# yukara-ikemiya/friendly-stable-audio-tools

Measured on NVIDIA H100. Metric: denoise_steps_per_s, higher is better.
Workload: dtype fp16 operands, fp32 accumulate (the reference's autocast dtype)

## Files before the change

friendly-stable-audio-tools_b200/csrc/gemm.cuh:

```cuda
#pragma once
#include "common.cuh"
#include "ptx.cuh"

namespace satb {

__device__ __forceinline__ int split_part(int idx, int n_parts) { return n_parts == 3 ? (idx == 2 ? 0 : idx + 1) : idx; }

struct GemmShape {
  int L;
  int batches;
  int N;
  int K;
  int n_taps;
  int tap_base;
  int tap_step;
  int b_tap_rows;
  int stride;
  int b_static = 0;
  int n_parts = 1;
  int b_part_rows = 0;
};

constexpr int kBlockM = 128;
constexpr int kBlockK = 64;
constexpr int kWgmmaK = 16;
constexpr int kGemmThreads = 384;
constexpr int kSmemBudget = 227 * 1024;

constexpr int kEpiWarps = 8;
template <int BN, int kCols, int kEpiStage = 0>
struct GemmCfg {
  static constexpr int kStageA = kBlockM * kBlockK * 2;
  static constexpr int kStageB = BN * kBlockK * 2;
  static constexpr int kStage = kStageA + kStageB;
  static constexpr int kAccLd = kCols + 4;
  static constexpr int kAccStage = 2 * 64 * kAccLd * 4;
  static constexpr int kFixed = 1024  + 256  + 2 * kAccStage + kEpiWarps * kEpiStage;
  static constexpr int kStages = (kSmemBudget - kFixed) / kStage > 8 ? 8 : (kSmemBudget - kFixed) / kStage;
  static constexpr int kSmemBytes = kStages * kStage + kFixed;
  static_assert(BN == 64 || BN == 128 || BN == 256, "BN must be 64/128/256");
  static_assert(kStages >= 2, "shared memory too small for a two-stage ring");
};

struct EpiCtx {
  int row;
  int l;
  int batch;
  int col0;
  bool valid;
  int l0;
  int L;
  int lane;
  float* stage;
};

template <class Epi, int BN>
__device__ __forceinline__ void gemm_tile_epilogue(const float (&acc)[BN / 2], float* acc_st, float* epi_st,
                                                   const typename Epi::Params& ep, int L, int N, int m0, int n0, int batch,
                                                   int cw, int warp, int lane) {
  const int wq = warp & 3;
  const int half = wq >> 1;
  const int rsub = (wq & 1) * 32;
  const int fr = 16 * wq + (lane >> 2);
  const int fc = 2 * (lane & 3);
  constexpr int kChunks = BN / Epi::kCols;
  constexpr int kLd = Epi::kCols + 4;
  EpiCtx c;
  c.l0 = m0 + 64 * cw + rsub;
  c.l = c.l0 + lane;
  c.batch = batch;
  c.row = batch * L + c.l;
  c.valid = c.l < L;
  c.L = L;
  c.lane = lane;
  c.stage = epi_st;
  int n_valid = (N - n0 + Epi::kCols - 1) / Epi::kCols;
  if (n_valid > kChunks) n_valid = kChunks;
#pragma unroll
  for (int cp = 0; cp < (kChunks + 1) / 2; ++cp) {
    named_bar_sync(1 + cw, 128);
#pragma unroll
    for (int hh = 0; hh < 2; ++hh) {
      const int ch = 2 * cp + hh;
      if (ch < kChunks) {
        float* dst = acc_st + hh * 64 * kLd;
#pragma unroll
        for (int j = 0; j < Epi::kCols / 8; ++j) {
          const int ai = (ch * (Epi::kCols / 8) + j) * 4;
          *reinterpret_cast<float2*>(dst + fr * kLd + 8 * j + fc) = make_float2(acc[ai], acc[ai + 1]);
          *reinterpret_cast<float2*>(dst + (fr + 8) * kLd + 8 * j + fc) = make_float2(acc[ai + 2], acc[ai + 3]);
        }
      }
    }
    named_bar_sync(1 + cw, 128);
    const int ci = 2 * cp + half;
    if (ci < n_valid) {
      uint32_t r[Epi::kCols];
      const float4* src = reinterpret_cast<const float4*>(acc_st + half * 64 * kLd + (rsub + lane) * kLd);
#pragma unroll
      for (int j = 0; j < Epi::kCols / 4; ++j) {
        const float4 v = src[j];
        r[4 * j] = __float_as_uint(v.x);
        r[4 * j + 1] = __float_as_uint(v.y);
        r[4 * j + 2] = __float_as_uint(v.z);
        r[4 * j + 3] = __float_as_uint(v.w);
      }
      c.col0 = n0 + ci * Epi::kCols;
      Epi::apply(ep, c, r);
    }
  }
}
template <class Epi, int BN, bool BF16>
__global__ void __launch_bounds__(kGemmThreads, 1)
gemm_wgmma_kernel(const __grid_constant__ CUtensorMap tmA, const __grid_constant__ CUtensorMap tmB,
                  const __grid_constant__ CUtensorMap tmA2, const GemmShape s, const typename Epi::Params ep) {
  using Cfg = GemmCfg<BN, Epi::kCols, Epi::kStageBytes>;
  extern __shared__ uint8_t smem_raw[];
  uint8_t* smem = reinterpret_cast<uint8_t*>((reinterpret_cast<uintptr_t>(smem_raw) + 1023) & ~uintptr_t(1023));
  uint64_t* bars = reinterpret_cast<uint64_t*>(smem + Cfg::kStages * Cfg::kStage);
  uint64_t* full_bar = bars;
  uint64_t* empty_bar = bars + Cfg::kStages;
  uint8_t* epi_smem = smem + Cfg::kStages * Cfg::kStage + 256;

  const int warp = threadIdx.x >> 5;
  const int lane = threadIdx.x & 31;
  const int wg = threadIdx.x >> 7;

  const int m_tiles = (s.L + kBlockM - 1) / kBlockM;
  const int n_tiles = (s.N + BN - 1) / BN;
  const int tiles_per_n = m_tiles * s.batches;
  const int total_tiles = tiles_per_n * n_tiles;
  const int kb_per_tap = (s.K + kBlockK - 1) / kBlockK;
  const int kb_per_part = kb_per_tap * s.n_taps;
  const int num_kb = kb_per_part * s.n_parts;

  if (threadIdx.x == 0) {
    tma_prefetch_desc(&tmA);
    tma_prefetch_desc(&tmB);
    for (int i = 0; i < Cfg::kStages; ++i) {
      mbar_init(&full_bar[i], 1);
      mbar_init(&empty_bar[i], 2);
    }
    fence_mbar_init();
  }
  __syncthreads();
  pdl_launch_dependents();

  if (wg == 0) {
    setmaxnreg_dec<40>();
    if (warp == 0 && elect_one()) {
      int pre = 0;
      if (s.b_static && static_cast<int>(blockIdx.x) < total_tiles) {
        pre = num_kb < Cfg::kStages ? num_kb : Cfg::kStages;
        const int n0 = (static_cast<int>(blockIdx.x) / tiles_per_n) * BN;
        for (int kb = 0; kb < pre; ++kb) {
          const int pidx = kb / kb_per_part, kbp = kb - pidx * kb_per_part;
          const int part = split_part(pidx, s.n_parts);
          const int tap = kbp / kb_per_tap;
          const int k0 = (kbp - tap * kb_per_tap) * kBlockK;
          mbar_expect_tx(&full_bar[kb], Cfg::kStage);
          tma_load_2d(smem + kb * Cfg::kStage + Cfg::kStageA, &tmB, &full_bar[kb], k0,
                      tap * s.b_tap_rows + n0 + (part == 2 ? s.b_part_rows : 0));
        }
      }
      pdl_wait();
      int stage = 0;
      uint32_t phase = 0;
      for (int tile = blockIdx.x; tile < total_tiles; tile += gridDim.x) {
        const int nt = tile / tiles_per_n;
        const int rem = tile - nt * tiles_per_n;
        const int batch = rem / m_tiles;
        const int m0 = (rem - batch * m_tiles) * kBlockM;
        const int n0 = nt * BN;
        for (int kb = 0; kb < num_kb; ++kb) {
          const int pidx = kb / kb_per_part, kbp = kb - pidx * kb_per_part;
          const int part = split_part(pidx, s.n_parts);
          const int tap = kbp / kb_per_tap;
          const int k0 = (kbp - tap * kb_per_tap) * kBlockK;
          mbar_wait(&empty_bar[stage], phase ^ 1);
          uint8_t* sa = smem + stage * Cfg::kStage;
          uint8_t* sb = sa + Cfg::kStageA;
          const bool b_done = tile == static_cast<int>(blockIdx.x) && kb < pre;
          if (!b_done) mbar_expect_tx(&full_bar[stage], Cfg::kStage);
          const int u = s.tap_base + tap * s.tap_step;
          int ph = 0, ro = u;
          if (s.stride > 1) {
            ro = (u >= 0) ? u / s.stride : -((-u + s.stride - 1) / s.stride);
            ph = u - ro * s.stride;
          }
          tma_load_4d(sa, part == 1 ? &tmA2 : &tmA, &full_bar[stage], k0, ph, m0 + ro, batch);
          if (!b_done)
            tma_load_2d(sb, &tmB, &full_bar[stage], k0, tap * s.b_tap_rows + n0 + (part == 2 ? s.b_part_rows : 0));
          if (++stage == Cfg::kStages) {
            stage = 0;
            phase ^= 1;
          }
        }
      }
    }
  } else {
    setmaxnreg_inc<232>();
    pdl_wait();
    const int cw = wg - 1;
    float* acc_st = reinterpret_cast<float*>(epi_smem + cw * Cfg::kAccStage);
    float* epi_st = Epi::kStageBytes > 0
                        ? reinterpret_cast<float*>(epi_smem + 2 * Cfg::kAccStage + (warp - 4) * Epi::kStageBytes)
                        : nullptr;
    float acc[BN / 2];
    int stage = 0;
    uint32_t phase = 0;
    for (int tile = blockIdx.x; tile < total_tiles; tile += gridDim.x) {
      const int nt = tile / tiles_per_n;
      const int rem = tile - nt * tiles_per_n;
      const int batch = rem / m_tiles;
      const int m0 = (rem - batch * m_tiles) * kBlockM;
      const int n0 = nt * BN;
      int prev = -1;
      for (int kb = 0; kb < num_kb; ++kb) {
        mbar_wait(&full_bar[stage], phase);
        const uint32_t a_addr = smem_u32(smem + stage * Cfg::kStage) + cw * 64 * kBlockK * 2;
        const uint32_t b_addr = smem_u32(smem + stage * Cfg::kStage) + Cfg::kStageA;
        wgmma_fence();
#pragma unroll
        for (int k = 0; k < kBlockK / kWgmmaK; ++k)
          wgmma_ss<BN, BF16>(acc, make_desc_kmajor_sw128(a_addr + k * kWgmmaK * 2),
                             make_desc_kmajor_sw128(b_addr + k * kWgmmaK * 2), (kb | k) != 0 ? 1u : 0u);
        wgmma_commit();
        wgmma_wait<1>(acc);
        if (prev >= 0 && (threadIdx.x & 127) == 0) mbar_arrive(&empty_bar[prev]);
        prev = stage;
        if (++stage == Cfg::kStages) {
          stage = 0;
          phase ^= 1;
        }
      }
      wgmma_wait<0>(acc);
      if ((threadIdx.x & 127) == 0) mbar_arrive(&empty_bar[prev]);

      gemm_tile_epilogue<Epi, BN>(acc, acc_st, epi_st, ep, s.L, s.N, m0, n0, batch, cw, warp, lane);
    }
  }
}


__device__ __forceinline__ float silu_f(float x) { return x / (1.0f + __expf(-x)); }

template <bool BF16>
struct EpiStore16 {
  static constexpr int kCols = 32;
  static constexpr int kStageBytes = 0;
  struct Params {
    void* out;
    int ld;
    const float* bias;
    int act;
  };
  __device__ static __forceinline__ void apply(const Params& p, const EpiCtx& c, const uint32_t (&r)[32]) {
    if (!c.valid) return;
    float v[32];
#pragma unroll
    for (int j = 0; j < 32; ++j) v[j] = __uint_as_float(r[j]);
    if (p.bias) {
#pragma unroll
      for (int j = 0; j < 32; j += 4) {
        const float4 b = __ldg(reinterpret_cast<const float4*>(p.bias + c.col0 + j));
        v[j] += b.x; v[j + 1] += b.y; v[j + 2] += b.z; v[j + 3] += b.w;
      }
    }
    uint32_t o[16];
#pragma unroll
    for (int j = 0; j < 16; ++j) {
      float a = v[2 * j], b = v[2 * j + 1];
      if (p.act == 1) {
        a = silu_f(a);
        b = silu_f(b);
      }
      o[j] = Op16<BF16>::pack(a, b);
    }
    uint4* dst = reinterpret_cast<uint4*>(static_cast<uint16_t*>(p.out) + static_cast<size_t>(c.row) * p.ld + c.col0);
#pragma unroll
    for (int j = 0; j < 4; ++j) dst[j] = make_uint4(o[4 * j], o[4 * j + 1], o[4 * j + 2], o[4 * j + 3]);
  }
};

struct EpiStore32 {
  static constexpr int kCols = 32;
  static constexpr int kStageBytes = 0;
  struct Params {
    float* out;
    int ld;
    const float* bias;
  };
  __device__ static __forceinline__ void apply(const Params& p, const EpiCtx& c, const uint32_t (&r)[32]) {
    if (!c.valid) return;
    float4* dst = reinterpret_cast<float4*>(p.out + static_cast<size_t>(c.row) * p.ld + c.col0);
#pragma unroll
    for (int j = 0; j < 8; ++j) {
      float4 v = make_float4(__uint_as_float(r[4 * j]), __uint_as_float(r[4 * j + 1]), __uint_as_float(r[4 * j + 2]),
                             __uint_as_float(r[4 * j + 3]));
      if (p.bias) {
        const float4 b = __ldg(reinterpret_cast<const float4*>(p.bias + c.col0) + j);
        v.x += b.x; v.y += b.y; v.z += b.z; v.w += b.w;
      }
      dst[j] = v;
    }
  }
};

struct EpiResidual {
  static constexpr int kCols = 32;
  static constexpr int kStageBytes = 0;
  struct Params {
    float* h;
    int ld;
    const float* bias;
    const float* gate;
    int rows_per_item;
    int gate_ld;
    int n_items;
  };
  __device__ static __forceinline__ void apply(const Params& p, const EpiCtx& c, const uint32_t (&r)[32]) {
    if (!c.valid) return;
    float4* dst = reinterpret_cast<float4*>(p.h + static_cast<size_t>(c.row) * p.ld + c.col0);
    const float4* g = p.gate ? reinterpret_cast<const float4*>(
                                   p.gate + static_cast<size_t>((c.row / p.rows_per_item) % p.n_items) * p.gate_ld + c.col0)
                             : nullptr;
#pragma unroll
    for (int j = 0; j < 8; ++j) {
      float4 v = make_float4(__uint_as_float(r[4 * j]), __uint_as_float(r[4 * j + 1]), __uint_as_float(r[4 * j + 2]),
                             __uint_as_float(r[4 * j + 3]));
      if (p.bias) {
        const float4 b = __ldg(reinterpret_cast<const float4*>(p.bias + c.col0) + j);
        v.x += b.x; v.y += b.y; v.z += b.z; v.w += b.w;
      }
      if (g) {
        const float4 gg = __ldg(g + j);
        v.x *= gg.x; v.y *= gg.y; v.z *= gg.z; v.w *= gg.w;
      }
      asm volatile("red.global.add.v4.f32 [%0], {%1, %2, %3, %4};" ::"l"(dst + j), "f"(v.x), "f"(v.y), "f"(v.z), "f"(v.w)
                   : "memory");
    }
  }
};

template <bool BF16>
struct EpiQkvRope {
  static constexpr int kCols = 32;
  static constexpr int kStageBytes = 0;
  struct Params {
    void* out;
    int ld;
    int rope_cols;
    int seq_len;
    int head_dim;
    int nf;
    const float* cos_tab;
    const float* sin_tab;
  };
  __device__ static __forceinline__ void apply(const Params& p, const EpiCtx& c, const uint32_t (&r)[32]) {
    if (!c.valid) return;
    float v[32];
#pragma unroll
    for (int j = 0; j < 32; ++j) v[j] = __uint_as_float(r[j]);
    const int ci = (c.col0 % p.head_dim) >> 5;
    const int n_rot = min(max(p.nf - 16 * ci, 0), 16);
    if (c.col0 < p.rope_cols && n_rot > 0 && p.cos_tab) {
      const int pos = c.row % p.seq_len;
      const float4* ct = reinterpret_cast<const float4*>(p.cos_tab + pos * p.nf + 16 * ci);
      const float4* st = reinterpret_cast<const float4*>(p.sin_tab + pos * p.nf + 16 * ci);
#pragma unroll
      for (int j4 = 0; j4 < 4; ++j4) {
        if (4 * j4 >= n_rot) break;
        const float4 cs = __ldg(ct + j4), sn = __ldg(st + j4);
        const float cc[4] = {cs.x, cs.y, cs.z, cs.w}, ss[4] = {sn.x, sn.y, sn.z, sn.w};
#pragma unroll
        for (int u = 0; u < 4; ++u) {
          const int j = j4 * 4 + u;
          const float a = v[j], b = v[j + 16];
          v[j] = a * cc[u] - b * ss[u];
          v[j + 16] = b * cc[u] + a * ss[u];
        }
      }
    }
    uint4* dst = reinterpret_cast<uint4*>(static_cast<uint16_t*>(p.out) + static_cast<size_t>(c.row) * p.ld + c.col0);
#pragma unroll
    for (int j = 0; j < 4; ++j)
      dst[j] = make_uint4(Op16<BF16>::pack(v[8 * j], v[8 * j + 1]), Op16<BF16>::pack(v[8 * j + 2], v[8 * j + 3]),
                          Op16<BF16>::pack(v[8 * j + 4], v[8 * j + 5]), Op16<BF16>::pack(v[8 * j + 6], v[8 * j + 7]));
  }
};

template <bool BF16>
struct EpiHeadNorm16 {
  static constexpr int kCols = 64;
  static constexpr int kStageBytes = 0;
  struct Params {
    void* out;
    int ld;
    int norm_cols;
    int rope_cols;
    int seq_len;
    const float* cos_tab;
    const float* sin_tab;
  };
  __device__ static __forceinline__ void apply(const Params& p, const EpiCtx& c, const uint32_t (&r)[64]) {
    if (!c.valid) return;
    float inv = 1.f;
    if (c.col0 < p.norm_cols) {
      float ss = 0.f;
#pragma unroll
      for (int j = 0; j < 64; ++j) ss = fmaf(__uint_as_float(r[j]), __uint_as_float(r[j]), ss);
      inv = 1.f / fmaxf(sqrtf(ss), 1e-12f);
    }
    uint4* dst = reinterpret_cast<uint4*>(static_cast<uint16_t*>(p.out) + static_cast<size_t>(c.row) * p.ld + c.col0);
    float v[32];
#pragma unroll
    for (int j = 0; j < 32; ++j) v[j] = __uint_as_float(r[j]) * inv;
    if (c.col0 < p.rope_cols && p.cos_tab) {
      const int pos = c.row % p.seq_len;
      const float4* ct = reinterpret_cast<const float4*>(p.cos_tab + pos * 16);
      const float4* st = reinterpret_cast<const float4*>(p.sin_tab + pos * 16);
#pragma unroll
      for (int j4 = 0; j4 < 4; ++j4) {
        const float4 cs = __ldg(ct + j4), sn = __ldg(st + j4);
        const float cc[4] = {cs.x, cs.y, cs.z, cs.w}, ss4[4] = {sn.x, sn.y, sn.z, sn.w};
#pragma unroll
        for (int u = 0; u < 4; ++u) {
          const int j = j4 * 4 + u;
          const float a = v[j], b = v[j + 16];
          v[j] = a * cc[u] - b * ss4[u];
          v[j + 16] = b * cc[u] + a * ss4[u];
        }
      }
    }
#pragma unroll
    for (int j = 0; j < 4; ++j)
      dst[j] = make_uint4(Op16<BF16>::pack(v[8 * j], v[8 * j + 1]), Op16<BF16>::pack(v[8 * j + 2], v[8 * j + 3]),
                          Op16<BF16>::pack(v[8 * j + 4], v[8 * j + 5]), Op16<BF16>::pack(v[8 * j + 6], v[8 * j + 7]));
#pragma unroll
    for (int j = 0; j < 4; ++j) {
      const uint32_t* q = &r[32 + 8 * j];
      dst[4 + j] = make_uint4(Op16<BF16>::pack(__uint_as_float(q[0]) * inv, __uint_as_float(q[1]) * inv),
                              Op16<BF16>::pack(__uint_as_float(q[2]) * inv, __uint_as_float(q[3]) * inv),
                              Op16<BF16>::pack(__uint_as_float(q[4]) * inv, __uint_as_float(q[5]) * inv),
                              Op16<BF16>::pack(__uint_as_float(q[6]) * inv, __uint_as_float(q[7]) * inv));
    }
  }
};

template <bool BF16>
struct EpiSwiglu {
  static constexpr int kCols = 64;
  static constexpr int kStageBytes = 0;
  struct Params {
    void* out;
    int ld;
    const float* bias;
  };
  __device__ static __forceinline__ void apply(const Params& p, const EpiCtx& c, const uint32_t (&r)[64]) {
    if (!c.valid) return;
    uint32_t o[16];
#pragma unroll
    for (int j = 0; j < 16; ++j) {
      float a0 = __uint_as_float(r[2 * j]), a1 = __uint_as_float(r[2 * j + 1]);
      float g0 = __uint_as_float(r[32 + 2 * j]), g1 = __uint_as_float(r[33 + 2 * j]);
      if (p.bias) {
        a0 += __ldg(p.bias + c.col0 + 2 * j);
        a1 += __ldg(p.bias + c.col0 + 2 * j + 1);
        g0 += __ldg(p.bias + c.col0 + 32 + 2 * j);
        g1 += __ldg(p.bias + c.col0 + 33 + 2 * j);
      }
      o[j] = Op16<BF16>::pack(a0 * silu_f(g0), a1 * silu_f(g1));
    }
    uint4* dst =
        reinterpret_cast<uint4*>(static_cast<uint16_t*>(p.out) + static_cast<size_t>(c.row) * p.ld + (c.col0 >> 1));
#pragma unroll
    for (int j = 0; j < 4; ++j) dst[j] = make_uint4(o[4 * j], o[4 * j + 1], o[4 * j + 2], o[4 * j + 3]);
  }
};

__device__ __forceinline__ float snake_fast(float v, float a, float ib) {
  const float sn = __sinf(v * a);
  return fmaf(ib, sn * sn, v);
}

__device__ __forceinline__ uint64_t f2_pack(float lo, float hi) {
  uint64_t d;
  asm("mov.b64 %0, {%1, %2};" : "=l"(d) : "f"(lo), "f"(hi));
  return d;
}
__device__ __forceinline__ void f2_unpack(uint64_t v, float& lo, float& hi) {
  asm("mov.b64 {%0, %1}, %2;" : "=f"(lo), "=f"(hi) : "l"(v));
}
__device__ __forceinline__ uint64_t f2_add(uint64_t a, uint64_t b) {
  float a0, a1, b0, b1;
  f2_unpack(a, a0, a1);
  f2_unpack(b, b0, b1);
  return f2_pack(__fadd_rn(a0, b0), __fadd_rn(a1, b1));
}
__device__ __forceinline__ uint64_t f2_mul(uint64_t a, uint64_t b) {
  float a0, a1, b0, b1;
  f2_unpack(a, a0, a1);
  f2_unpack(b, b0, b1);
  return f2_pack(__fmul_rn(a0, b0), __fmul_rn(a1, b1));
}
__device__ __forceinline__ uint64_t f2_fma(uint64_t a, uint64_t b, uint64_t c) {
  float a0, a1, b0, b1, c0, c1;
  f2_unpack(a, a0, a1);
  f2_unpack(b, b0, b1);
  f2_unpack(c, c0, c1);
  return f2_pack(__fmaf_rn(a0, b0, c0), __fmaf_rn(a1, b1, c1));
}
__device__ __forceinline__ uint64_t snake_fast2(uint64_t v, uint64_t a, uint64_t ib) {
  float t0, t1;
  f2_unpack(f2_mul(v, a), t0, t1);
  const uint64_t sn = f2_pack(__sinf(t0), __sinf(t1));
  return f2_fma(ib, f2_mul(sn, sn), v);
}

struct EpiConvParams {
  const float* bias;
  const void* resid;
  void* raw_out;
  void* s16_out;
  const float* sn_a;
  const float* sn_ib;
  int cout;
  int L_out;
  int up;
  int pad;
  void* s16_lo_out;
  int raw16;
};
template <bool BF16, bool MASKED = false>
struct EpiConv {
  static constexpr int kCols = 32;
  static constexpr int kStageBytes = 32 * 36 * 4;
  typedef EpiConvParams Params;
  __host__ __device__ static bool fast_flags(const Params& p) {
    return p.s16_out != nullptr && p.sn_a != nullptr && p.s16_lo_out == nullptr &&
           (p.raw16 != 0 || (p.resid == nullptr && p.raw_out == nullptr));
  }
  struct Seg {
    int phase, co;
  };
  __device__ static __forceinline__ Seg seg_of(const Params& p, const EpiCtx& c) {
    Seg sg{0, c.col0};
    if (p.up > 1) {
      sg.phase = c.col0 / p.cout;
      sg.co = c.col0 - sg.phase * p.cout;
    }
    sg.co += 4 * (c.lane & 7);
    return sg;
  }
  __device__ static __forceinline__ bool seg_index(const Params& p, const EpiCtx& c, const Seg& sg, int i, size_t* idx) {
    const int l = c.l0 + (c.lane >> 3) + 4 * i;
    const int lo = l * p.up + sg.phase - p.pad;
    const bool ok = l < c.L && lo >= 0 && lo < p.L_out;
    *idx = (static_cast<size_t>(c.batch) * p.L_out + (ok ? lo : 0)) * p.cout + sg.co;
    return ok;
  }
  struct Plan {
    long long idx0;
    int stride;
    uint32_t mask;
    int co;
  };
  __device__ static __forceinline__ Plan chunk_plan(const Params& p, const EpiCtx& c) {
    const Seg sg = seg_of(p, c);
    const int l0 = c.l0 + (c.lane >> 3);
    const int lo0 = l0 * p.up + sg.phase - p.pad;
    Plan pl;
    pl.mask = 0;
#pragma unroll
    for (int i = 0; i < 8; ++i) {
      const int l = l0 + 4 * i, lo = lo0 + 4 * i * p.up;
      if (l < c.L && lo >= 0 && lo < p.L_out) pl.mask |= 1u << i;
    }
    pl.idx0 = (static_cast<long long>(c.batch) * p.L_out + lo0) * p.cout + sg.co;
    pl.stride = 4 * p.up * p.cout;
    pl.co = sg.co;
    return pl;
  }
  __device__ static __forceinline__ void prefetch_masked(const Params& p, const EpiCtx& c, float4 (&rs)[8]) {
    if (p.resid) {
      const Plan pl = chunk_plan(p, c);
      const uint16_t* rp = static_cast<const uint16_t*>(p.resid) + pl.idx0;
#pragma unroll
      for (int i = 0; i < 8; ++i) {
        uint2 u = make_uint2(0u, 0u);
        if ((pl.mask >> i) & 1u) u = *reinterpret_cast<const uint2*>(rp);
        rp += pl.stride;
        rs[i] = make_float4(__uint_as_float(u.x), __uint_as_float(u.y), 0.f, 0.f);
      }
    }
  }
  template <bool RESID, bool RAWOUT>
  __device__ static __forceinline__ void finish_masked_t(const Params& p, const EpiCtx& c, const uint32_t (&r)[32],
                                                         const float4 (&rs)[8]) {
    const Plan pl = chunk_plan(p, c);
    const uint32_t st = smem_u32(c.stage);
    const int g = c.lane & 7, r0 = c.lane >> 3;
#pragma unroll
    for (int j = 0; j < 8; ++j) sts128(st + (c.lane * 36 + 4 * j) * 4, r[4 * j], r[4 * j + 1], r[4 * j + 2], r[4 * j + 3]);
    __syncwarp();
    ulonglong2 b2 = make_ulonglong2(0ull, 0ull);
    if (p.bias) b2 = __ldg(reinterpret_cast<const ulonglong2*>(p.bias + pl.co));
    const ulonglong2 a2 = __ldg(reinterpret_cast<const ulonglong2*>(p.sn_a + pl.co));
    const ulonglong2 ib2 = __ldg(reinterpret_cast<const ulonglong2*>(p.sn_ib + pl.co));
    uint16_t* raw_o = static_cast<uint16_t*>(p.raw_out) + pl.idx0;
    uint16_t* s_o = static_cast<uint16_t*>(p.s16_out) + pl.idx0;
    uint32_t ld_addr = st + (r0 * 36 + 4 * g) * 4;
#pragma unroll
    for (int i = 0; i < 8; ++i) {
      const ulonglong2 acc = lds128_b64x2(ld_addr);
      ld_addr += 4 * 36 * 4;
      const bool ok = (pl.mask >> i) & 1u;
      uint64_t v01 = f2_add(acc.x, b2.x), v23 = f2_add(acc.y, b2.y);
      if (RESID) {
        const float2 lo = Op16<BF16>::unpack(__float_as_uint(rs[i].x)), hi = Op16<BF16>::unpack(__float_as_uint(rs[i].y));
        v01 = f2_add(v01, f2_pack(lo.x, lo.y));
        v23 = f2_add(v23, f2_pack(hi.x, hi.y));
      }
      if (RAWOUT) {
        float y0, y1, y2, y3;
        f2_unpack(v01, y0, y1);
        f2_unpack(v23, y2, y3);
        if (ok) *reinterpret_cast<uint2*>(raw_o) = make_uint2(Op16<BF16>::pack(y0, y1), Op16<BF16>::pack(y2, y3));
        raw_o += pl.stride;
      }
      v01 = snake_fast2(v01, a2.x, ib2.x);
      v23 = snake_fast2(v23, a2.y, ib2.y);
      float x0, x1, x2, x3;
      f2_unpack(v01, x0, x1);
      f2_unpack(v23, x2, x3);
      if (ok) *reinterpret_cast<uint2*>(s_o) = make_uint2(Op16<BF16>::pack(x0, x1), Op16<BF16>::pack(x2, x3));
      s_o += pl.stride;
    }
    __syncwarp();
  }
  __device__ static __forceinline__ void finish_masked(const Params& p, const EpiCtx& c, const uint32_t (&r)[32],
                                                       const float4 (&rs)[8]) {
    if (p.resid) {
      if (p.raw_out) finish_masked_t<true, true>(p, c, r, rs);
      else finish_masked_t<true, false>(p, c, r, rs);
    } else {
      if (p.raw_out) finish_masked_t<false, true>(p, c, r, rs);
      else finish_masked_t<false, false>(p, c, r, rs);
    }
  }
  __device__ static __forceinline__ void prefetch(const Params& p, const EpiCtx& c, float4 (&rs)[8]) {
    if constexpr (MASKED) {
      prefetch_masked(p, c, rs);
      return;
    }
    const Seg sg = seg_of(p, c);
#pragma unroll
    for (int i = 0; i < 8; ++i) {
      size_t idx;
      const bool ok = seg_index(p, c, sg, i, &idx);
      rs[i] = make_float4(0.f, 0.f, 0.f, 0.f);
      if (ok && p.resid) {
        if (p.raw16) {
          const uint2 u = *reinterpret_cast<const uint2*>(static_cast<const uint16_t*>(p.resid) + idx);
          rs[i] = make_float4(__uint_as_float(u.x), __uint_as_float(u.y), 0.f, 0.f);
        } else {
          rs[i] = *reinterpret_cast<const float4*>(static_cast<const float*>(p.resid) + idx);
        }
      }
    }
  }
  __device__ static __forceinline__ void finish(const Params& p, const EpiCtx& c, const uint32_t (&r)[32],
                                                const float4 (&rs)[8]) {
    if constexpr (MASKED) {
      finish_masked(p, c, r, rs);
      return;
    }
    float* st = c.stage;
    const int g = c.lane & 7, r0 = c.lane >> 3;
    {
      float4* mine = reinterpret_cast<float4*>(st + c.lane * 36);
#pragma unroll
      for (int j = 0; j < 8; ++j)
        mine[j] = make_float4(__uint_as_float(r[4 * j]), __uint_as_float(r[4 * j + 1]), __uint_as_float(r[4 * j + 2]),
                              __uint_as_float(r[4 * j + 3]));
    }
    __syncwarp();
    const Seg sg = seg_of(p, c);
    const int co = sg.co;
    ulonglong2 b2 = make_ulonglong2(0ull, 0ull), a2 = b2, ib2 = b2;
    if (p.bias) b2 = __ldg(reinterpret_cast<const ulonglong2*>(p.bias + co));
    const bool snake = p.s16_out != nullptr && p.sn_a != nullptr;
    if (snake) {
      a2 = __ldg(reinterpret_cast<const ulonglong2*>(p.sn_a + co));
      ib2 = __ldg(reinterpret_cast<const ulonglong2*>(p.sn_ib + co));
    }
#pragma unroll
    for (int i = 0; i < 8; ++i) {
      size_t idx;
      if (seg_index(p, c, sg, i, &idx)) {
        const ulonglong2 acc = *reinterpret_cast<const ulonglong2*>(st + (r0 + 4 * i) * 36 + 4 * g);
        uint64_t r01, r23;
        if (p.raw16 && p.resid) {
          const float2 lo = Op16<BF16>::unpack(__float_as_uint(rs[i].x)), hi = Op16<BF16>::unpack(__float_as_uint(rs[i].y));
          r01 = f2_pack(lo.x, lo.y);
          r23 = f2_pack(hi.x, hi.y);
        } else {
          r01 = f2_pack(rs[i].x, rs[i].y);
          r23 = f2_pack(rs[i].z, rs[i].w);
        }
        uint64_t v01 = f2_add(acc.x, f2_add(b2.x, r01));
        uint64_t v23 = f2_add(acc.y, f2_add(b2.y, r23));
        if (p.raw_out) {
          if (p.raw16) {
            float y0, y1, y2, y3;
            f2_unpack(v01, y0, y1);
            f2_unpack(v23, y2, y3);
            *reinterpret_cast<uint2*>(static_cast<uint16_t*>(p.raw_out) + idx) =
                make_uint2(Op16<BF16>::pack(y0, y1), Op16<BF16>::pack(y2, y3));
          } else {
            *reinterpret_cast<ulonglong2*>(static_cast<float*>(p.raw_out) + idx) = make_ulonglong2(v01, v23);
          }
        }
        if (p.s16_out) {
          if (snake) {
            v01 = snake_fast2(v01, a2.x, ib2.x);
            v23 = snake_fast2(v23, a2.y, ib2.y);
          }
          float x0, x1, x2, x3;
          f2_unpack(v01, x0, x1);
          f2_unpack(v23, x2, x3);
          const uint32_t h01 = Op16<BF16>::pack(x0, x1), h23 = Op16<BF16>::pack(x2, x3);
          *reinterpret_cast<uint2*>(static_cast<uint16_t*>(p.s16_out) + idx) = make_uint2(h01, h23);
          if (p.s16_lo_out) {
            const float2 a = Op16<BF16>::unpack(h01), b = Op16<BF16>::unpack(h23);
            *reinterpret_cast<uint2*>(static_cast<uint16_t*>(p.s16_lo_out) + idx) =
                make_uint2(Op16<BF16>::pack(x0 - a.x, x1 - a.y), Op16<BF16>::pack(x2 - b.x, x3 - b.y));
          }
        }
      }
    }
    __syncwarp();
  }
  __device__ static __forceinline__ void apply(const Params& p, const EpiCtx& c, const uint32_t (&r)[32]) {
    float4 rs[8];
    prefetch(p, c, rs);
    finish(p, c, r, rs);
  }
};

struct EpiStoreNCL {
  static constexpr int kCols = 32;
  static constexpr int kStageBytes = 0;
  struct Params {
    float* out;
    const float* bias;
    int N;
    int L;
    int do_tanh;
  };
  __device__ static __forceinline__ void apply(const Params& p, const EpiCtx& c, const uint32_t (&r)[32]) {
    if (!c.valid) return;
    float* o = p.out + (static_cast<size_t>(c.batch) * p.N + c.col0) * p.L + c.l;
#pragma unroll
    for (int j = 0; j < 32; ++j) {
      if (c.col0 + j < p.N) {
        const float v = __uint_as_float(r[j]) + (p.bias ? __ldg(p.bias + c.col0 + j) : 0.f);
        o[static_cast<size_t>(j) * p.L] = p.do_tanh ? tanhf(v) : v;
      }
    }
  }
};

int make_tmap_a(CUtensorMap* m, const void* ptr, int K, int L, int batches, int64_t row_stride_elems,
                int64_t batch_stride_elems, int stride = 1, int box_rows = kBlockM);
int make_tmap_b(CUtensorMap* m, const void* ptr, int K, int rows, int64_t row_stride_elems, int box_rows);

template <class Epi, int BN, bool BF16>
int launch_gemm(const CUtensorMap& tmA, const CUtensorMap& tmB, const GemmShape& s, const typename Epi::Params& ep,
                cudaStream_t stream, const CUtensorMap* tmA2 = nullptr) {
  using Cfg = GemmCfg<BN, Epi::kCols, Epi::kStageBytes>;
  auto kern = gemm_wgmma_kernel<Epi, BN, BF16>;
  static PerDeviceOnce attr;
  if (attr.first()) SATB_CHECK_CUDA(cudaFuncSetAttribute(kern, cudaFuncAttributeMaxDynamicSharedMemorySize, Cfg::kSmemBytes));
  const int m_tiles = ceil_div(s.L, kBlockM), n_tiles = ceil_div(s.N, BN);
  const int total = m_tiles * s.batches * n_tiles;
  if (total <= 0) return 0;
  int grid = device_sm_count();
  if (grid > total) grid = total;
  SATB_REQUIRE(s.n_parts == 1 || tmA2 != nullptr, "split-operand GEMM needs the second A tensor map");
  SATB_CHECK_CUDA(launch_pdl(kern, dim3(grid), dim3(kGemmThreads), Cfg::kSmemBytes, stream, tmA, tmB, tmA2 ? *tmA2 : tmA, s, ep));
  count_launch();
  return 0;
}

}
```

Measured before the change: 24.87.

## Apply residual and SwiGLU epilogues directly from WGMMA register fragments

Adds a fragment-epilogue path in which EpiResidual and EpiSwiglu consume the WGMMA accumulator registers directly, so the accumulator no longer round-trips through shared memory. Kernels using these epilogues drop the accumulator staging area, which frees shared memory for more pipeline stages. In exchange, global stores and reductions become narrower and less coalesced (v2 reductions and 32-bit stores per lane instead of v4/uint4 rows), and the swiglu path now depends on the gate columns sitting in the same fragment.

```diff
diff --git a/friendly-stable-audio-tools_b200/csrc/gemm.cuh b/friendly-stable-audio-tools_b200/csrc/gemm.cuh
--- a/friendly-stable-audio-tools_b200/csrc/gemm.cuh
+++ b/friendly-stable-audio-tools_b200/csrc/gemm.cuh
@@ -1,4 +1,6 @@
 #pragma once
+#include <type_traits>
+
 #include "common.cuh"
 #include "ptx.cuh"
 
@@ -34,13 +36,20 @@
   static constexpr int kStageB = BN * kBlockK * 2;
   static constexpr int kStage = kStageA + kStageB;
   static constexpr int kAccLd = kCols + 4;
-  static constexpr int kAccStage = 2 * 64 * kAccLd * 4;
+  static constexpr int kAccStage = kCols ? 2 * 64 * kAccLd * 4 : 0;
   static constexpr int kFixed = 1024  + 256  + 2 * kAccStage + kEpiWarps * kEpiStage;
   static constexpr int kStages = (kSmemBudget - kFixed) / kStage > 8 ? 8 : (kSmemBudget - kFixed) / kStage;
   static constexpr int kSmemBytes = kStages * kStage + kFixed;
   static_assert(BN == 64 || BN == 128 || BN == 256, "BN must be 64/128/256");
   static_assert(kStages >= 2, "shared memory too small for a two-stage ring");
 };
+
+template <class Epi, class = void>
+struct EpiFragment : std::false_type {};
+template <class Epi>
+struct EpiFragment<Epi, std::void_t<decltype(Epi::kFragment)>> : std::bool_constant<Epi::kFragment> {};
+template <class Epi>
+constexpr int kStagedCols = EpiFragment<Epi>::value ? 0 : Epi::kCols;
 
 struct EpiCtx {
   int row;
@@ -114,7 +123,7 @@
 __global__ void __launch_bounds__(kGemmThreads, 1)
 gemm_wgmma_kernel(const __grid_constant__ CUtensorMap tmA, const __grid_constant__ CUtensorMap tmB,
                   const __grid_constant__ CUtensorMap tmA2, const GemmShape s, const typename Epi::Params ep) {
-  using Cfg = GemmCfg<BN, Epi::kCols, Epi::kStageBytes>;
+  using Cfg = GemmCfg<BN, kStagedCols<Epi>, Epi::kStageBytes>;
   extern __shared__ uint8_t smem_raw[];
   uint8_t* smem = reinterpret_cast<uint8_t*>((reinterpret_cast<uintptr_t>(smem_raw) + 1023) & ~uintptr_t(1023));
   uint64_t* bars = reinterpret_cast<uint64_t*>(smem + Cfg::kStages * Cfg::kStage);
@@ -237,7 +246,10 @@
       wgmma_wait<0>(acc);
       if ((threadIdx.x & 127) == 0) mbar_arrive(&empty_bar[prev]);
 
-      gemm_tile_epilogue<Epi, BN>(acc, acc_st, epi_st, ep, s.L, s.N, m0, n0, batch, cw, warp, lane);
+      if constexpr (EpiFragment<Epi>::value)
+        Epi::template apply_fragment<BN>(ep, acc, s.L, s.N, m0 + 64 * cw + 16 * (warp & 3) + (lane >> 2), n0, batch, lane);
+      else
+        gemm_tile_epilogue<Epi, BN>(acc, acc_st, epi_st, ep, s.L, s.N, m0, n0, batch, cw, warp, lane);
     }
   }
 }
@@ -310,6 +322,7 @@
 struct EpiResidual {
   static constexpr int kCols = 32;
   static constexpr int kStageBytes = 0;
+  static constexpr bool kFragment = true;
   struct Params {
     float* h;
     int ld;
@@ -319,26 +332,36 @@
     int gate_ld;
     int n_items;
   };
-  __device__ static __forceinline__ void apply(const Params& p, const EpiCtx& c, const uint32_t (&r)[32]) {
-    if (!c.valid) return;
-    float4* dst = reinterpret_cast<float4*>(p.h + static_cast<size_t>(c.row) * p.ld + c.col0);
-    const float4* g = p.gate ? reinterpret_cast<const float4*>(
-                                   p.gate + static_cast<size_t>((c.row / p.rows_per_item) % p.n_items) * p.gate_ld + c.col0)
-                             : nullptr;
-#pragma unroll
-    for (int j = 0; j < 8; ++j) {
-      float4 v = make_float4(__uint_as_float(r[4 * j]), __uint_as_float(r[4 * j + 1]), __uint_as_float(r[4 * j + 2]),
-                             __uint_as_float(r[4 * j + 3]));
-      if (p.bias) {
-        const float4 b = __ldg(reinterpret_cast<const float4*>(p.bias + c.col0) + j);
-        v.x += b.x; v.y += b.y; v.z += b.z; v.w += b.w;
-      }
-      if (g) {
-        const float4 gg = __ldg(g + j);
-        v.x *= gg.x; v.y *= gg.y; v.z *= gg.z; v.w *= gg.w;
-      }
-      asm volatile("red.global.add.v4.f32 [%0], {%1, %2, %3, %4};" ::"l"(dst + j), "f"(v.x), "f"(v.y), "f"(v.z), "f"(v.w)
-                   : "memory");
+  template <int BN>
+  __device__ static __forceinline__ void apply_fragment(const Params& p, const float (&acc)[BN / 2], int L, int N,
+                                                        int row0, int n0, int batch, int lane) {
+    const int fc = 2 * (lane & 3);
+    const float* grow[2] = {nullptr, nullptr};
+    float* hrow[2];
+#pragma unroll
+    for (int rr = 0; rr < 2; ++rr) {
+      const int row = batch * L + row0 + 8 * rr;
+      hrow[rr] = p.h + static_cast<size_t>(row) * p.ld + n0 + fc;
+      if (p.gate) grow[rr] = p.gate + static_cast<size_t>((row / p.rows_per_item) % p.n_items) * p.gate_ld + n0 + fc;
+    }
+#pragma unroll
+    for (int j = 0; j < BN / 8; ++j) {
+      if (n0 + 8 * j >= N) break;
+      float2 b = make_float2(0.f, 0.f);
+      if (p.bias) b = __ldg(reinterpret_cast<const float2*>(p.bias + n0 + fc + 8 * j));
+#pragma unroll
+      for (int rr = 0; rr < 2; ++rr) {
+        if (row0 + 8 * rr >= L) continue;
+        float2 v = make_float2(acc[4 * j + 2 * rr], acc[4 * j + 2 * rr + 1]);
+        if (p.bias) {
+          v.x += b.x; v.y += b.y;
+        }
+        if (p.gate) {
+          const float2 gg = __ldg(reinterpret_cast<const float2*>(grow[rr] + 8 * j));
+          v.x *= gg.x; v.y *= gg.y;
+        }
+        asm volatile("red.global.add.v2.f32 [%0], {%1, %2};" ::"l"(hrow[rr] + 8 * j), "f"(v.x), "f"(v.y) : "memory");
+      }
     }
   }
 };
@@ -452,30 +475,45 @@
 struct EpiSwiglu {
   static constexpr int kCols = 64;
   static constexpr int kStageBytes = 0;
+  static constexpr bool kFragment = true;
   struct Params {
     void* out;
     int ld;
     const float* bias;
   };
-  __device__ static __forceinline__ void apply(const Params& p, const EpiCtx& c, const uint32_t (&r)[64]) {
-    if (!c.valid) return;
-    uint32_t o[16];
-#pragma unroll
-    for (int j = 0; j < 16; ++j) {
-      float a0 = __uint_as_float(r[2 * j]), a1 = __uint_as_float(r[2 * j + 1]);
-      float g0 = __uint_as_float(r[32 + 2 * j]), g1 = __uint_as_float(r[33 + 2 * j]);
-      if (p.bias) {
-        a0 += __ldg(p.bias + c.col0 + 2 * j);
-        a1 += __ldg(p.bias + c.col0 + 2 * j + 1);
-        g0 += __ldg(p.bias + c.col0 + 32 + 2 * j);
-        g1 += __ldg(p.bias + c.col0 + 33 + 2 * j);
-      }
-      o[j] = Op16<BF16>::pack(a0 * silu_f(g0), a1 * silu_f(g1));
-    }
-    uint4* dst =
-        reinterpret_cast<uint4*>(static_cast<uint16_t*>(p.out) + static_cast<size_t>(c.row) * p.ld + (c.col0 >> 1));
-#pragma unroll
-    for (int j = 0; j < 4; ++j) dst[j] = make_uint4(o[4 * j], o[4 * j + 1], o[4 * j + 2], o[4 * j + 3]);
+  template <int BN>
+  __device__ static __forceinline__ void apply_fragment(const Params& p, const float (&acc)[BN / 2], int L, int N,
+                                                        int row0, int n0, int batch, int lane) {
+    const int fc = 2 * (lane & 3);
+#pragma unroll
+    for (int g = 0; g < BN / 64; ++g) {
+      const int col0 = n0 + 64 * g;
+      if (col0 >= N) break;
+#pragma unroll
+      for (int jj = 0; jj < 4; ++jj) {
+        const int c = 8 * jj + fc;
+        float2 bv = make_float2(0.f, 0.f), bg = bv;
+        if (p.bias) {
+          bv = __ldg(reinterpret_cast<const float2*>(p.bias + col0 + c));
+          bg = __ldg(reinterpret_cast<const float2*>(p.bias + col0 + 32 + c));
+        }
+#pragma unroll
+        for (int rr = 0; rr < 2; ++rr) {
+          const int l = row0 + 8 * rr;
+          if (l >= L) continue;
+          const int av = 4 * (8 * g + jj) + 2 * rr, ag = av + 16;
+          float a0 = acc[av], a1 = acc[av + 1], g0 = acc[ag], g1 = acc[ag + 1];
+          if (p.bias) {
+            a0 += bv.x;
+            a1 += bv.y;
+            g0 += bg.x;
+            g1 += bg.y;
+          }
+          uint16_t* dst = static_cast<uint16_t*>(p.out) + static_cast<size_t>(batch * L + l) * p.ld + (col0 >> 1) + c;
+          *reinterpret_cast<uint32_t*>(dst) = Op16<BF16>::pack(a0 * silu_f(g0), a1 * silu_f(g1));
+        }
+      }
+    }
   }
 };
 
@@ -779,7 +817,7 @@
 template <class Epi, int BN, bool BF16>
 int launch_gemm(const CUtensorMap& tmA, const CUtensorMap& tmB, const GemmShape& s, const typename Epi::Params& ep,
                 cudaStream_t stream, const CUtensorMap* tmA2 = nullptr) {
-  using Cfg = GemmCfg<BN, Epi::kCols, Epi::kStageBytes>;
+  using Cfg = GemmCfg<BN, kStagedCols<Epi>, Epi::kStageBytes>;
   auto kern = gemm_wgmma_kernel<Epi, BN, BF16>;
   static PerDeviceOnce attr;
   if (attr.first()) SATB_CHECK_CUDA(cudaFuncSetAttribute(kern, cudaFuncAttributeMaxDynamicSharedMemorySize, Cfg::kSmemBytes));
```

Result: faster. 26.10, median of 6 (+4.9%).
